# hguo/ftk

Measured on NVIDIA B200. Metric: space_time_simplices_tested_per_sec, higher is better.
Workload: dtype f64+int64

## Files before the change

### ftk_b200/csrc/context.cpp

```cpp
#include <algorithm>
#include <cfloat>
#include <chrono>
#include <cmath>
#include <cstdio>
#include <cstdlib>
#include <cstring>
#include <deque>
#include <string>
#include <thread>
#include <atomic>
#include <vector>

#include <future>
#include <memory>
#include "kernels.h"
#include "online.h"
#include "curves.h"

using namespace ftkb;

namespace {

thread_local std::string g_create_error;

// ... 19 lines not shown
};
template <class T> using RawVec = std::vector<T, NoInitAlloc<T>>;

struct ftkb_ctx {
  ftkb_config cfg{};
  int n = 0;
  size_t nvert = 0;
  uint64_t ncore = 0;
  int n_ord = 0, n_int = 0;
  cudaStream_t stream = nullptr;
  cudaEvent_t ev[8] = {nullptr, nullptr, nullptr, nullptr, nullptr, nullptr, nullptr, nullptr};
  bool derive_timed = false;
  std::string error;

  bool slab = false;
  void *d_f32 = nullptr;
  size_t f32_cap = 0;
  std::deque<Layer> layers;
  std::vector<double *> freeS, freeV, freeJ;
  int current_timestep = 0;
  double resolution = DBL_MAX;
  double factor = 1.0;
  int nbits = 0;
  int next_slot = 0;
  int sm_count = 148;
  int scan_mode = 2;
  bool cellsV = true;
  bool cells2d = true;
  bool keys2d = true;
  bool cells3d = true;
  std::vector<uint4 *> freeCells;
  std::vector<uint4 *> exportedCells;
  size_t ncells = 0;
  bool fused3d = false;

  unsigned long long *d_scalars = nullptr;
  unsigned long long *h_scalars = nullptr;
  static constexpr int SLOT_WL = 8, SLOT_PT = 9, SLOT_UQ = 10, SLOT_POISON = 11, SLOT_WL2 = 12, SLOT_TICKET = 13, SLOT_POISON2 = 14, NSLOTS = 16;

  struct Pending {
    int ring = 0, evset = 0, pops = 0, nbits = 0, wl_sel = 0;
    uint64_t seq = 0, npts_before = 0, pt_cap = 0;
    bool has_next = false;
    int res_slots[2] = {-1, -1};
  };
  bool defer = true;
  std::deque<Pending> pend;
  std::deque<Layer> limbo;
  unsigned long long *h_ring = nullptr;
  static constexpr int RING = 4;
  uint64_t step_seq = 0;
  bool primed = false;
  int wl_sel = 0;
  cudaEvent_t dev[2][3] = {{nullptr, nullptr, nullptr}, {nullptr, nullptr, nullptr}};
  bool push_d2h_outstanding = false;
  uint64_t wl_hint = 1 << 16;
  cudaEvent_t ev_input = nullptr;
  cudaStream_t producer = nullptr;
  cudaStream_t stream2 = nullptr;
  cudaEvent_t ev_join = nullptr;
  bool debug_timing = false;
  double gap_ms = 0; uint64_t gap_n = 0, last_confirmed_seq = 0;
  std::vector<float> gaps, tl_scan_end, tl_test_end;
  cudaEvent_t dbg_prev = nullptr; bool dbg_prev_valid = false;
  double host_wait_us = 0, host_enq_us = 0; uint64_t host_wait_n = 0, host_enq_n = 0;
  bool overlap_test = true;
// ... 590 lines not shown
static void fused3d_decomposition(const ftkb_ctx *c, SweepParams &p, bool cells = false) {
  p.nsx = (p.W + F3_STRIDE - 1) / F3_STRIDE;
  p.nsy = (p.H + F3_TROWS - 1) / F3_TROWS;
  const int64_t tiles = (int64_t)p.nsx * p.nsy;
  if (c->cells3d || cells) {
    const int64_t slots = 2 * (int64_t)c->sm_count;
    const int64_t nsz = std::max<int64_t>(1, std::min<int64_t>((6 * slots + tiles - 1) / tiles, std::max(1, p.D / 16)));
    p.rows = (int)((p.D + nsz - 1) / nsz);
    if (const char *e = std::getenv("FTKB_S3_ROWS")) p.rows = std::max(1, std::min(p.D, std::atoi(e)));
    p.rows = std::min(p.rows, 63);
    p.nsz = (p.D + p.rows - 1) / p.rows;
    return;
  }
  int64_t nsz = std::max<int64_t>(1, (2 * (int64_t)c->sm_count) / tiles);
  nsz = std::min<int64_t>(nsz, std::max(1, p.D / 8));
  p.rows = (int)((p.D + nsz - 1) / nsz);
  p.nsz = (p.D + p.rows - 1) / p.rows;
}

static void vcells_decomposition(const ftkb_ctx *c, SweepParams &p) {
  if (c->n == 3) { fused3d_decomposition(c, p, true); return; }
  const int R = VSCAN2D_CELL_ROWS;
  p.nsx = std::max(1, (p.W + 61) / 62);
  const int64_t want = std::max<int64_t>(1, (6 * (int64_t)c->sm_count * 16) / p.nsx);
  p.rows = std::max(2 * R, (int)((p.H + want - 1) / want));
  p.rows = (p.rows + R - 1) / R * R;
  if (const char *e = std::getenv("FTKB_V2_ROWS")) p.rows = std::max(R, std::atoi(e) / R * R);
  p.nsy = (p.H + p.rows - 1) / p.rows;
  p.nsz = 1;
}

static int ensure_cells(ftkb_ctx *c, Layer &l, const SweepParams &p) {
  if (l.cells) return FTKB_OK;
  if (!c->ncells) c->ncells = c->n == 3 ? scan3d_cells_per_layer(p) : (p.fused ? scan2d_cells_per_layer(p) : vscan2d_cells_per_layer(p));
  if (!c->freeCells.empty()) { l.cells = c->freeCells.back(); c->freeCells.pop_back(); return FTKB_OK; }
  CK(cudaMalloc(&l.cells, sizeof(uint4) * c->ncells));
  return FTKB_OK;
}

static int materialise_gradient(ftkb_ctx *c, Layer &l) {
  if (l.V || !l.S) return FTKB_OK;
  CK(cudaMemsetAsync(c->d_scalars + l.slot, 0xff, sizeof(unsigned long long), c->stream));
  int rc = take_buffer(c, c->freeV, c->nvert * c->n, &l.V);
  if (rc) return rc;
  l.ownV = true;
  l.cells_valid = false;
  launch_gradient(c->n, l.S, l.V, c->cfg.dims[0], c->cfg.dims[1], c->n == 3 ? c->cfg.dims[2] : 1, c->d_scalars + l.slot, c->stream);
  c->stats.kernel_launches++;
  l.res_pending = false;
  CK(cudaMemcpyAsync(c->h_scalars + l.slot, c->d_scalars + l.slot, sizeof(unsigned long long), cudaMemcpyDeviceToHost, c->stream));
  c->stats.d2h_bytes += 8;
  c->push_d2h_outstanding = true;
  return check_launch(c, "gradient");
}

static int abandon_fused3d(ftkb_ctx *c) {
  c->fused3d = false;
  for (Layer &l : c->layers) {
    const int rc = materialise_gradient(c, l);
    if (rc) return rc;
  }
  CK(cudaStreamSynchronize(c->stream));
  return FTKB_OK;
}

static bool rows_aligned16(const ftkb_ctx *c, const double *a, const double *b) {
  return (c->cfg.dims[0] % 2 == 0) && ((uintptr_t)a % 16 == 0) && (!b || (uintptr_t)b % 16 == 0);
}

// ... 1025 lines not shown
  std::memcpy(out->bytes, &h, 64);
  out->offset = (uint64_t)((uintptr_t)dev_ptr - (uintptr_t)base);
  return FTKB_OK;
}

extern "C" int ftkb_ipc_import(const ftkb_ipc_handle *h, int device, void **dev_ptr) {
  if (!h || !dev_ptr) return FTKB_ERR_INVALID;
  if (cudaSetDevice(device) != cudaSuccess) { cudaGetLastError(); return FTKB_ERR_NO_DEVICE; }
  cudaIpcMemHandle_t ih;
  std::memcpy(&ih, h->bytes, 64);
  void *base = nullptr;
  if (cudaIpcOpenMemHandle(&base, ih, cudaIpcMemLazyEnablePeerAccess) != cudaSuccess) { cudaGetLastError(); return FTKB_ERR_CUDA; }
  *dev_ptr = static_cast<char *>(base) + h->offset;
  return FTKB_OK;
}

extern "C" int ftkb_ipc_close(void *dev_ptr, const ftkb_ipc_handle *h) {
  if (!dev_ptr || !h) return FTKB_ERR_INVALID;
  if (cudaIpcCloseMemHandle(static_cast<char *>(dev_ptr) - h->offset) != cudaSuccess) { cudaGetLastError(); return FTKB_ERR_CUDA; }
  return FTKB_OK;
}

extern "C" int ftkb_export_layer_cells(ftkb_ctx *c, int index, void **cells, uint64_t *bytes, double *resolution) {
  if (!c || !cells || !bytes) return FTKB_ERR_INVALID;
  if (index < 0 || (size_t)index >= c->layers.size()) return fail(c, FTKB_ERR_INVALID, "export_layer_cells: no such resident layer");
  { const int rc = drain(c); if (rc) return rc; }
  if ((size_t)index >= c->layers.size()) return fail(c, FTKB_ERR_INVALID, "export_layer_cells: no such resident layer");
  Layer &l = c->layers[index];
  if (!l.cells || !l.cells_valid) return fail(c, FTKB_ERR_INVALID, "export_layer_cells: the layer has no range cells yet (a sweep must have read it)");
  CK(cudaSetDevice(c->cfg.device));
  CK(cudaStreamSynchronize(c->stream));
  if (!l.cells_foreign) { l.cells_foreign = true; c->exportedCells.push_back(l.cells); }
  *cells = l.cells;
  *bytes = (uint64_t)c->ncells * sizeof(uint4);
  if (resolution) *resolution = l.res_pending ? DBL_MAX : slot_value(c, l.slot);
  return FTKB_OK;
}

extern "C" int ftkb_push_snapshot_remote(ftkb_ctx *c, const double *scalar, const double *vector, const void *cells, double resolution) {
  if (!c || !cells || (!scalar && !vector)) return FTKB_ERR_INVALID;
  if (c->cfg.jacobian_source == FTKB_SOURCE_GIVEN) return fail(c, FTKB_ERR_INVALID, "push_snapshot_remote: a GIVEN jacobian cannot be remote");
  if (c->cfg.vector_source == FTKB_SOURCE_GIVEN ? !vector : !scalar) return fail(c, FTKB_ERR_INVALID, "push_snapshot_remote: the field the sweep reads is missing");
  CK(cudaSetDevice(c->cfg.device));
  if ((uintptr_t)scalar % 8 != 0 || (uintptr_t)vector % 8 != 0 || (uintptr_t)cells % 16 != 0)
    return fail(c, FTKB_ERR_INVALID, "push_snapshot_remote: arrays must be 8-byte aligned, cells 16-byte aligned");
  Layer l;
  int rc = new_layer(c, l);
  if (rc) return rc;
  l.S = const_cast<double *>(scalar);
  l.V = const_cast<double *>(vector);
  l.cells = reinterpret_cast<uint4 *>(const_cast<void *>(cells));
  l.cells_valid = true;
  l.cells_foreign = true;
  l.res_pending = false;
  unsigned long long bits;
  const double r = resolution > 0 ? resolution : DBL_MAX;
  std::memcpy(&bits, &r, 8);
  if (!(resolution > 0) || resolution >= DBL_MAX) bits = ~0ull;
  c->h_scalars[l.slot] = bits;
  CK(cudaMemcpyAsync(c->d_scalars + l.slot, c->h_scalars + l.slot, sizeof(unsigned long long), cudaMemcpyHostToDevice, c->stream));
  c->layers.push_back(l);
  return FTKB_OK;
}

extern "C" int ftkb_get_curveset(ftkb_ctx *c, ftkb_curveset **out) {
  if (!c || !out) return FTKB_ERR_INVALID;
  if (!c->traced) return fail(c, FTKB_ERR_INVALID, "get_curveset: call finalize first");
// ... 203 lines not shown
```

### ftk_b200/csrc/kernels.cu

```cuda
#include "kernels.h"

#include <algorithm>
#include <cfloat>
#include <cstdlib>
#include <string>
#include <climits>
#include <cub/device/device_radix_sort.cuh>
#include <cub/device/device_select.cuh>

namespace ftkb {

typedef long long i64;
typedef unsigned long long u64;

__constant__ DeviceMeshTables c_mesh[2];

void upload_mesh_tables(const DeviceMeshTables &t2, const DeviceMeshTables &t3) {
  DeviceMeshTables h[2] = {t2, t3};
  cudaMemcpyToSymbol(c_mesh, h, sizeof(h));
}

constexpr int KEY_ONE = 0x3FF00000;
constexpr int KEY_POISON_EXP = 0x43E00000;

// ... 758 lines not shown
      const int col_lo = max(C0 - 2, 0), col_hi = min(C0 - 2 + TL_SEG, W);
      const uint32_t seg_bytes = (uint32_t)(col_hi - col_lo) * 8u;
      const uint32_t dst0 = smem_u32(ring) + (uint32_t)(col_lo - (C0 - 2)) * 8u;
      for (int rr = 0; rr < nrows; rr++) {
        const int st = rr % TL_NST;
        if (rr >= TL_NST) mbar_wait(empty0 + 8u * st, (uint32_t)((rr / TL_NST - 1) & 1));
        const size_t off = (size_t)W * (size_t)clampi(r0 - 1 + rr, H) + (size_t)col_lo;
        mbar_expect_tx(full0 + 8u * st, seg_bytes * NL);
#pragma unroll
        for (int L = 0; L < NL; L++)
          bulk_g2s(dst0 + (uint32_t)st * STAGE_BYTES + (uint32_t)(L * TL_SEG) * 8u, (L == 0 ? p.L[0].S : p.L[1].S) + off, seg_bytes, full0 + 8u * st);
      }
    }
    return;
  }
  if (wib >= nactive) return;
  const int c0 = C0 + wib * FB_STRIDE;
  const double *tile = ring + wib * FB_STRIDE;
  const bool border = c0 == 0 || c0 + FB_SEG - 2 > W || (p.ub[0] >= c0 - 1 && p.ub[0] <= c0 + 63);
  if (border) fused2d_tile_strip<HAS_NEXT, true>(p, c0, r0, r1, lane, tile, full0, empty0);
  else fused2d_tile_strip<HAS_NEXT, false>(p, c0, r0, r1, lane, tile, full0, empty0);
}

constexpr int C2_R = 9;
constexpr int C2_NST = 9;
constexpr int C2_CW = TL_CW;
static_assert(C2_R % 3 == 0 && C2_R == C2_NST && C2_R == SCAN2D_CELL_ROWS, "row window / ring / cell block must stay aligned");

__device__ __forceinline__ size_t cells2d_index(const SweepParams &p, const int strip, const int kb, const int lane) {
  const size_t nblk = (size_t)(p.H / C2_R + 2);
  return ((size_t)strip * nblk + (size_t)kb) * 32u + (size_t)lane;
}

template <int NL>
__device__ __forceinline__ void cells2d_slow_cubes_t(const SweepParams &p, unsigned failmask, const int c0, const int y0, const int nrows, const uint32_t stage) {
  static_assert(2 * C2_R <= 32, "one lane per cube");
  const int W = p.W, H = p.H;
  const int lane = threadIdx.x & 31;
  const float cwf = (float)(W - 1), chf = (float)(H - 1);
  const float nanf_ = __int_as_float(0x7FC00000);
  const int per = 2 * nrows, total = per * __popc(failmask);
  for (int q0 = 0; q0 < total; q0 += 32) {
    const int qi = q0 + lane;
    const bool live = qi < total;
    const int which = live ? qi / per : 0, within = live ? qi % per : 0;
    const int src = (int)__fns(failmask, 0, which + 1);
    const int r = within >> 1, q = within & 1;
    const int x = c0 + 2 * src + q, y = y0 + r;
    const bool in = live && x >= p.lb[0] && x <= p.ub[0] && y >= p.lb[1] && y <= p.ub[1];
    const int xs[4] = {clampi(x - 1, W), clampi(x, W), clampi(x + 1, W), clampi(x + 2, W)};
    size_t rows_[4];
#pragma unroll
    for (int k = 0; k < 4; k++) rows_[k] = (size_t)W * (size_t)clampi(y - 1 + k, H);
    FRange rx{nanf_, nanf_}, ry{nanf_, nanf_};
#pragma unroll
    for (int L = 0; L < NL; L++) {
      const double *S = p.L[L].S;
      double h[2][4], lo[2], hi[2];
#pragma unroll
      for (int j = 0; j < 2; j++)
#pragma unroll
        for (int k = 0; k < 4; k++) h[j][k] = __ldg(S + rows_[1 + j] + xs[k]);
#pragma unroll
      for (int i = 0; i < 2; i++) { lo[i] = __ldg(S + rows_[0] + xs[1 + i]); hi[i] = __ldg(S + rows_[3] + xs[1 + i]); }
#pragma unroll
      for (int v = 0; v < 4; v++) {
// ... 5 lines not shown
        rx = fmerge(rx, FRange{fx, fx}); ry = fmerge(ry, FRange{fy, fy});
      }
    }
    const bool surv = in && !cube_excluded2_f(rx, ry, p.thrp_f, p.thr2_f, p.lim_f);
    const u64 lin = (u64)(x - p.lb[0]) + (u64)p.nc[0] * (u64)(y - p.lb[1]);
    if (stage) stage_survivors(p, stage, surv, lin);
    else append_survivors(p, surv, lin);
  }
}
__device__ __noinline__ void cells2d_slow_cubes(const SweepParams &p, unsigned failmask, const int c0, const int y0, const int nl, const int nrows, const uint32_t stage = 0) {
  if (nl == 1) cells2d_slow_cubes_t<1>(p, failmask, c0, y0, nrows, stage);
  else cells2d_slow_cubes_t<2>(p, failmask, c0, y0, nrows, stage);
}

__device__ __forceinline__ void cells2d_decide(const SweepParams &p, const FRange ux, const FRange uy, const bool own, const int e, const int y0, const int nl) {
  const bool fail = own && !cube_excluded2_f(ux, uy, p.thrp_f, p.thr2_f, p.lim_f);
  const unsigned fm = __ballot_sync(0xffffffffu, fail);
  if (fm) cells2d_slow_cubes(p, fm, e - 2 * (int)(threadIdx.x & 31), y0, nl, C2_R);
}

template <bool BORDER, int NPREV, bool TEST>
__device__ __forceinline__ void cells2d_strip(const SweepParams &p, const int c0, const int r0, const int r1, const int lane,
                                              const double *tile , const uint32_t full0, const uint32_t empty0,
                                              const int strip) {
  const int W = p.W, H = p.H, B = p.build_layer;
  const int e = c0 + 2 * lane, o = e + 1;
  const bool e_in = !BORDER || e < W, o_in = !BORDER || o < W, o1_in = !BORDER || o + 1 < W;
  const bool own_cols = lane <= 30 && ((e >= p.lb[0] && e <= p.ub[0]) || (o >= p.lb[0] && o <= p.ub[0]));
  const int jl = r1 + 1;
  const float cwf = (float)(W - 1), chf = (float)(H - 1);
  const bool want_res = p.res_slot[B] != nullptr;
  double rmin = DBL_MAX;
  float rminf = 3.4028234e38f;
  const uint4 *sum_prev = NPREV ? p.sum_in[0] + cells2d_index(p, strip, 0, lane) : nullptr;
  uint4 *sum_out = p.sum_out + cells2d_index(p, strip, 0, lane);

  const double *lane_base = tile + 2 * lane;
  auto centre = [&](const int st, double (&dst)[2]) {
    const double2 t = *reinterpret_cast<const double2 *>(lane_base + st * TL_SEG + 2);
    dst[0] = t.x; dst[1] = t.y;
  };
  auto release = [&](const int st) {
    __syncwarp();
    if (elect_one()) mbar_arrive(empty0 + 8u * st);
  };
  auto finish_block = [&](const int kb, FRange bx, FRange by, const uint4 prevc) {
    bx = fmerge(bx, fshfl_down1(bx));
    by = fmerge(by, fshfl_down1(by));
    sum_out[(size_t)kb * 32u] = make_uint4(__float_as_uint(bx.mn), __float_as_uint(bx.mx), __float_as_uint(by.mn), __float_as_uint(by.mx));
    if (TEST) {
      if (NPREV) {
        bx = fmerge(bx, FRange{__uint_as_float(prevc.x), __uint_as_float(prevc.y)});
        by = fmerge(by, FRange{__uint_as_float(prevc.z), __uint_as_float(prevc.w)});
      }
      const int y0 = kb * C2_R;
      const bool own = own_cols && y0 <= p.ub[1] && y0 + C2_R - 1 >= p.lb[1];
      cells2d_decide(p, bx, by, own, e, y0, NPREV + 1);
    }
  };

  double win[3][2];
  mbar_wait(full0, 0);
  centre(0, win[0]);
  mbar_wait(full0 + 8, 0);
  centre(1, win[1]);
  release(0);
  FRange bx{0.f, 0.f}, by{0.f, 0.f};
  uint4 prevc = make_uint4(0x7FC00000u, 0x7FC00000u, 0x7FC00000u, 0x7FC00000u);

  auto step = [&](auto KC, const int j, const int i) {
    constexpr int K = decltype(KC)::value;
    constexpr int ST_J = (1 + K) % C2_NST, ST_P = (2 + K) % C2_NST;
    double (&m1)[2] = win[K % 3];
    double (&c0v)[2] = win[(K + 1) % 3];
    double (&p1)[2] = win[(K + 2) % 3];
    mbar_wait(full0 + 8u * ST_P, (uint32_t)((i + (2 + K >= C2_NST ? 1 : 0)) & 1));
    centre(ST_P, p1);
    const double *rowj = lane_base + ST_J * TL_SEG;
    double left = rowj[1], right = rowj[4];
    double mid_e = c0v[1];
    if (BORDER) {
      if (e == 0) left = c0v[0];
      if (!o_in) mid_e = c0v[0];
      if (!o1_in) right = c0v[1];
    }
    const double dxe = mid_e - left, dxo = right - c0v[0], dye = p1[0] - m1[0], dyo = p1[1] - m1[1];
    const float fxe = __double2float_rn(dxe) * cwf, fxo = __double2float_rn(dxo) * cwf;
    const float fye = __double2float_rn(dye) * chf, fyo = __double2float_rn(dyo) * chf;
    if (want_res && j < H) {
      float a = fminf(fminf(fabsf(fxe), fabsf(fye)), fminf(fabsf(fxo), fabsf(fyo)));
      if (BORDER) a = fminf(e_in ? fminf(fabsf(fxe), fabsf(fye)) : 3.4028234e38f, o_in ? fminf(fabsf(fxo), fabsf(fyo)) : 3.4028234e38f);
      if (a < rminf) res_update4(rmin, rminf, e_in, o_in, dxe, dye, dxo, dyo, (double)(W - 1), (double)(H - 1));
    }
    const FRange rx{fminf(fxe, fxo), fmaxf(fxe, fxo)}, ry{fminf(fye, fyo), fmaxf(fye, fyo)};
    if (K == 0) {
      if (j > r0) finish_block(j / C2_R - 1, fmerge(bx, rx), fmerge(by, ry), prevc);
      bx = rx; by = ry;
      if (NPREV && j < jl) prevc = __ldg(sum_prev + (size_t)(j / C2_R) * 32u);
    } else {
      bx = fmerge(bx, rx); by = fmerge(by, ry);
    }
// ... 44 lines not shown
      const uint32_t seg_bytes = (uint32_t)(col_hi - col_lo) * 8u;
      const uint32_t dst0 = smem_u32(ring) + (uint32_t)(col_lo - (C0 - 2)) * 8u;
      for (int rr = 0; rr < nrows; rr++) {
        const int st = rr % C2_NST;
        if (rr >= C2_NST) mbar_wait(empty0 + 8u * st, (uint32_t)((rr / C2_NST - 1) & 1));
        const size_t off = (size_t)W * (size_t)clampi(r0 - 1 + rr, H) + (size_t)col_lo;
        mbar_expect_tx(full0 + 8u * st, seg_bytes);
        bulk_g2s(dst0 + (uint32_t)st * STAGE_BYTES, S + off, seg_bytes, full0 + 8u * st);
      }
    }
    return;
  }
  if (wib >= nactive) return;
  const int c0 = C0 + wib * FB_STRIDE;
  const double *tile = ring + wib * FB_STRIDE;
  const bool border = c0 == 0 || c0 + FB_SEG - 2 > W;
  if (border) cells2d_strip<true, NPREV, TEST>(p, c0, r0, r1, lane, tile, full0, empty0, bx * C2_CW + wib);
  else cells2d_strip<false, NPREV, TEST>(p, c0, r0, r1, lane, tile, full0, empty0, bx * C2_CW + wib);
}

template <int NL>
__global__ void __launch_bounds__(256) scan2d_cells_kernel(const __grid_constant__ SweepParams p, const int nstrips, const int nblk_used) {
  const int lane = threadIdx.x & 31;
  const long long w = (long long)blockIdx.x * 8 + (threadIdx.x >> 5);
  if (w >= (long long)nstrips * nblk_used) return;
  const int strip = (int)(w / nblk_used), kb = (int)(w % nblk_used);
  const int e = strip * FB_STRIDE + 2 * lane, y0 = kb * C2_R;
  const bool own = lane <= 30 && ((e >= p.lb[0] && e <= p.ub[0]) || (e + 1 >= p.lb[0] && e + 1 <= p.ub[0])) && y0 <= p.ub[1] && y0 + C2_R - 1 >= p.lb[1];
  if (!__any_sync(0xffffffffu, own)) return;
  const float nanf_ = __int_as_float(0x7FC00000);
  FRange ux{nanf_, nanf_}, uy{nanf_, nanf_};
#pragma unroll
  for (int L = 0; L < NL; L++) {
    const uint4 c = __ldg(p.sum_in[L] + cells2d_index(p, strip, kb, lane));
    ux = fmerge(ux, FRange{__uint_as_float(c.x), __uint_as_float(c.y)});
    uy = fmerge(uy, FRange{__uint_as_float(c.z), __uint_as_float(c.w)});
  }
  cells2d_decide(p, ux, uy, own, e, y0, NL);
}

constexpr int K2_R = 3;
constexpr uint32_t K2_ROW_BYTES = TL_SEG * 8;
constexpr uint32_t K2_STAGE_BYTES = K2_R * K2_ROW_BYTES;
static_assert(C2_R % K2_R == 0, "cell block = whole stages");

__device__ __forceinline__ double2 lds128_f64(uint32_t a) {
  double2 v;
  asm volatile("ld.shared.v2.f64 {%0, %1}, [%2];" : "=d"(v.x), "=d"(v.y) : "r"(a));
  return v;
}
__device__ __forceinline__ double lds64_f64(uint32_t a) {
  double v;
  asm volatile("ld.shared.f64 %0, [%1];" : "=d"(v) : "r"(a));
  return v;
}
__device__ __forceinline__ void cp_async16(uint32_t dst, const void *src) {
  asm volatile("cp.async.cg.shared.global [%0], [%1], 16;" ::"r"(dst), "l"(src) : "memory");
}
__device__ __forceinline__ void cp_async_wait_all() { asm volatile("cp.async.wait_all;" ::: "memory"); }
__device__ __forceinline__ void cp_async_commit() { asm volatile("cp.async.commit_group;" ::: "memory"); }
template <int N> __device__ __forceinline__ void cp_async_wait_group() { asm volatile("cp.async.wait_group %0;" ::"n"(N) : "memory"); }
__device__ __forceinline__ uint4 lds128_u32(uint32_t a) {
  uint4 v;
  asm volatile("ld.shared.v4.u32 {%0, %1, %2, %3}, [%4];" : "=r"(v.x), "=r"(v.y), "=r"(v.z), "=r"(v.w) : "r"(a) : "memory");
  return v;
}
__device__ __forceinline__ void sts64_f64(uint32_t a, double v) { asm volatile("st.shared.f64 [%0], %1;" ::"r"(a), "d"(v) : "memory"); }
__device__ __forceinline__ float fmax_nan(float a, float b) {
  float r;
  asm("max.NaN.f32 %0, %1, %2;" : "=f"(r) : "f"(a), "f"(b));
  return r;
}

__device__ __forceinline__ double nzmin(double m, double d) {
  double r;
  asm("{\n\t.reg .pred p, q;\n\t.reg .f64 ad, am;\n\tabs.f64 ad, %2;\n\tabs.f64 am, %1;\n\t"
      "setp.neu.f64 q, %2, 0d0000000000000000;\n\tsetp.lt.and.f64 p, ad, am, q;\n\tselp.f64 %0, %2, %1, p;\n\t}"
      : "=d"(r) : "d"(m), "d"(d));
  return r;
}

__device__ __forceinline__ FRange k2_vrange(float kmn, float kmx, double c) {
  const int a = __float_as_int(kmn), b = __float_as_int(kmx);
  const double lo = __hiloint2double(a < 0 ? a + 1 : a, 0);
  const double hi = __hiloint2double(b < 0 ? b : b + 1, 0);
  return FRange{__double2float_rd(lo * c), __double2float_ru(hi * c)};
}

__device__ __forceinline__ void prefetch_l2(const void *q) { asm volatile("prefetch.global.L2 [%0];" ::"l"(q)); }

struct K2Acc { double mdx, mdy; float big; };

template <bool BORDER, int NPREV, bool TEST, int K2_NST>
__device__ __forceinline__ K2Acc keys2d_strip(const SweepParams &p, const int c0, const int r0, const int r1, const int lane,
                                           const uint32_t tile_u32 ,
                                           const uint32_t full0, const uint32_t empty0, const int strip,
                                           const uint32_t sbase ,
                                           const uint32_t res_u32 ,
                                           const uint32_t wl_stage ,
                                           const uint32_t cell_stage ,
                                           const K2Acc acc) {
  float big = acc.big;
  const int W = p.W, H = p.H, B = p.build_layer;
  const int e = c0 + 2 * lane, o = e + 1;
  const bool e_in = !BORDER || e < W, o_in = !BORDER || o < W, o1_in = !BORDER || o + 1 < W;
  const bool own_cols = lane <= 30 && ((e >= p.lb[0] && e <= p.ub[0]) || (o >= p.lb[0] && o <= p.ub[0]));
  const int jl = r1 + 1;
  const int nrows = jl - r0 + 1;
  const int ngroups = (nrows + K2_R - 1) / K2_R, nstages = (nrows + 2 + K2_R - 1) / K2_R;
  const double cw = (double)(W - 1), ch = (double)(H - 1);
  const bool want_res = p.res_slot[B] != nullptr;
  const float thrx = p.res_thr[0], thry = p.res_thr[1];
  const uint4 *sum_prev = NPREV ? p.sum_in[0] + cells2d_index(p, strip, 0, lane) : nullptr;
  uint4 *sum_out = p.sum_out + cells2d_index(p, strip, 0, lane);
  const uint32_t lane_u32 = tile_u32 + (uint32_t)lane * 16u;
  const int kb0 = r0 / C2_R;
  unsigned long long failbits = 0;
  const int kb_end = ((r1 + 1) + C2_R - 1) / C2_R;

  auto finish_block = [&](const int kb, float xmn, float xmx, float ymn, float ymx) {
    xmn = fminf(xmn, __shfl_down_sync(0xffffffffu, xmn, 1)); xmx = fmaxf(xmx, __shfl_down_sync(0xffffffffu, xmx, 1));
    ymn = fminf(ymn, __shfl_down_sync(0xffffffffu, ymn, 1)); ymx = fmaxf(ymx, __shfl_down_sync(0xffffffffu, ymx, 1));
    FRange bx = k2_vrange(xmn, xmx, cw), by = k2_vrange(ymn, ymx, ch);
    sum_out[(size_t)kb * 32u] = make_uint4(__float_as_uint(bx.mn), __float_as_uint(bx.mx), __float_as_uint(by.mn), __float_as_uint(by.mx));
    if (TEST) {
      if (NPREV && kb < kb_end) {
        cp_async_wait_all();
        const uint4 prevc = lds128_u32(cell_stage + ((uint32_t)kb & 1u) * 512u);
        bx = fmerge(bx, FRange{__uint_as_float(prevc.x), __uint_as_float(prevc.y)});
        by = fmerge(by, FRange{__uint_as_float(prevc.z), __uint_as_float(prevc.w)});
      }
      const int y0 = kb * C2_R;
      const bool own = own_cols && y0 <= p.ub[1] && y0 + C2_R - 1 >= p.lb[1];
      if (own && !cube_excluded2_f(bx, by, p.thrp_f, p.thr2_f, p.lim_f)) failbits |= 1ull << (kb - kb0);
    }
  };

  double C[2][K2_R][2];
  float KX[2][K2_R][2];
  auto load_stage = [&](auto PC, const int s) {
    constexpr int P = decltype(PC)::value;
    const uint32_t gs = sbase + (uint32_t)s, slot = gs % K2_NST;
    mbar_wait(full0 + 8u * slot, (gs / K2_NST) & 1u);
    const uint32_t base = lane_u32 + slot * K2_STAGE_BYTES;
    double nl[K2_R], nr[K2_R];
#pragma unroll
    for (int i = 0; i < K2_R; i++) {
      const double2 c = lds128_f64(base + (uint32_t)i * K2_ROW_BYTES + 16u);
      C[P][i][0] = c.x; C[P][i][1] = c.y;
      nl[i] = lds64_f64(base + (uint32_t)i * K2_ROW_BYTES + 8u);
      nr[i] = lds64_f64(base + (uint32_t)i * K2_ROW_BYTES + 32u);
    }
    float ax = __int_as_float(0x7F800000);
#pragma unroll
    for (int i = 0; i < K2_R; i++) {
      const float ke = fabsf(hikey(C[P][i][0])), ko = fabsf(hikey(C[P][i][1]));
      big = fmax_nan(big, BORDER ? (e_in ? ke : 0.f) : ke);
      big = fmax_nan(big, BORDER ? (o_in ? ko : 0.f) : ko);
      double left = nl[i], right = nr[i], mid_e = C[P][i][1];
      if (BORDER) {
        if (e == 0) left = C[P][i][0];
        if (!o_in) mid_e = C[P][i][0];
        if (!o1_in) right = C[P][i][1];
      }
      const double dxe = mid_e - left, dxo = right - C[P][i][0];
      KX[P][i][0] = hikey(dxe); KX[P][i][1] = hikey(dxo);
      ax = fminf(ax, fminf(fabsf(KX[P][i][0]), fabsf(KX[P][i][1])));
    }
    if (want_res && __any_sync(0xffffffffu, ax <= thrx)) {
      double mdx = lds64_f64(res_u32);
#pragma unroll
      for (int i = 0; i < K2_R; i++) {
        const int j = r0 + K2_R * s + i - 1;
        if (j >= r0 && j <= jl && j < H) {
          double left = lds64_f64(base + (uint32_t)i * K2_ROW_BYTES + 8u), right = lds64_f64(base + (uint32_t)i * K2_ROW_BYTES + 32u), mid_e = C[P][i][1];
          if (BORDER) {
            if (e == 0) left = C[P][i][0];
            if (!o_in) mid_e = C[P][i][0];
            if (!o1_in) right = C[P][i][1];
          }
          if (e_in) mdx = nzmin(mdx, mid_e - left);
          if (o_in) mdx = nzmin(mdx, right - C[P][i][0]);
        }
      }
      sts64_f64(res_u32, mdx);
    }
    __syncwarp();
    if (elect_one()) mbar_arrive(empty0 + 8u * slot);
  };

  float bxmn = 0.f, bxmx = 0.f, bymn = 0.f, bymx = 0.f;
  const uint4 nanc = make_uint4(0x7FC00000u, 0x7FC00000u, 0x7FC00000u, 0x7FC00000u);
  int kb = r0 / C2_R;
  if (NPREV && kb < kb_end) prefetch_l2(sum_prev + (size_t)kb * 32u);
  if (NPREV && kb + 1 < kb_end) prefetch_l2(sum_prev + (size_t)(kb + 1) * 32u);

  int gphase = 0;
  static_assert(C2_R == 3 * K2_R, "a cell block is three groups");
  auto group = [&](auto PC, const int g) {
    constexpr int P = decltype(PC)::value;
    if (g + 1 < nstages) load_stage(IC<1 - P>{}, g + 1);
    const bool opens_group = gphase == 0;
    gphase = gphase == 2 ? 0 : gphase + 1;
    const int j0 = r0 + K2_R * g;
    const bool full = j0 + K2_R - 1 <= min(jl, H - 1);
    float ay = __int_as_float(0x7F800000);
#pragma unroll
    for (int i = 0; i < K2_R; i++) {
      const int j = j0 + i;
      if (!full && j > jl) break;
      const double *m1 = C[P][i];
      const float *kx = i + 1 < K2_R ? KX[P][i + 1] : KX[1 - P][i + 1 - K2_R];
      const double *p1 = i + 2 < K2_R ? C[P][i + 2] : C[1 - P][i + 2 - K2_R];
      const double dye = p1[0] - m1[0], dyo = p1[1] - m1[1];
      const float kxe = kx[0], kxo = kx[1], kye = hikey(dye), kyo = hikey(dyo);
      ay = fminf(ay, fminf(fabsf(kye), fabsf(kyo)));
      if (i == 0 && opens_group) {
        const float rxmn = fminf(kxe, kxo), rxmx = fmaxf(kxe, kxo), rymn = fminf(kye, kyo), rymx = fmaxf(kye, kyo);
        if (j > r0) finish_block(kb - 1, fminf(bxmn, rxmn), fmaxf(bxmx, rxmx), fminf(bymn, rymn), fmaxf(bymx, rymx));
        bxmn = rxmn; bxmx = rxmx; bymn = rymn; bymx = rymx;
        if (NPREV && kb < kb_end) cp_async16(cell_stage + ((uint32_t)kb & 1u) * 512u, sum_prev + (size_t)kb * 32u);
        kb++;
        if (NPREV && kb + 1 < kb_end) prefetch_l2(sum_prev + (size_t)(kb + 1) * 32u);
      } else {
        bxmn = fminf(fminf(bxmn, kxe), kxo); bxmx = fmaxf(fmaxf(bxmx, kxe), kxo);
        bymn = fminf(fminf(bymn, kye), kyo); bymx = fmaxf(fmaxf(bymx, kye), kyo);
      }
    }
    if (want_res && __any_sync(0xffffffffu, ay <= thry)) {
      double mdy = lds64_f64(res_u32 + 8u);
#pragma unroll
      for (int i = 0; i < K2_R; i++) {
        const int j = j0 + i;
        if (!full && (j > jl || j >= H)) break;
        const double *m1 = C[P][i];
        const double *p1 = i + 2 < K2_R ? C[P][i + 2] : C[1 - P][i + 2 - K2_R];
        if (e_in) mdy = nzmin(mdy, p1[0] - m1[0]);
        if (o_in) mdy = nzmin(mdy, p1[1] - m1[1]);
      }
      sts64_f64(res_u32 + 8u, mdy);
    }
  };

  load_stage(IC<0>{}, 0);
#pragma unroll 1
  for (int g = 0; g < ngroups; g += 2) {
    group(IC<0>{}, g);
    if (g + 1 < ngroups) group(IC<1>{}, g + 1);
  }
  if (jl % C2_R != 0) finish_block(jl / C2_R, bxmn, bxmx, bymn, bymx);
  if (TEST) {
    for (int b = 0; b < 64; b++) {
      if (!__any_sync(0xffffffffu, (failbits >> b) != 0)) break;
      const unsigned fm = __ballot_sync(0xffffffffu, (failbits >> b) & 1ull);
// ... 75 lines not shown
    const char *e = std::getenv("FTKB_K2_CTAS"), *n = std::getenv("FTKB_K2_NST");
    const int ctas = e ? std::atoi(e) : 3, nst = n ? std::atoi(n) : 4;
    if (ctas == 2) return 28;
    if (ctas == 4) return 44;
    return nst == 5 ? 35 : (nst == 6 ? 36 : 34);
  }();
  return v;
}
template <int CTAS, int NST>
static void k2_launch(const SweepParams &p, unsigned grid, cudaStream_t s) {
  const size_t sm = k2_smem_bytes(NST);
  switch (p.sum_mode) {
    case SUM_BUILD: scan2d_keys_build_kernel<0, false, CTAS, NST><<<grid, (C2_CW + 1) * 32, sm, s>>>(p); break;
    case SUM_BUILD_TEST1: scan2d_keys_build_kernel<0, true, CTAS, NST><<<grid, (C2_CW + 1) * 32, sm, s>>>(p); break;
    default: scan2d_keys_build_kernel<1, true, CTAS, NST><<<grid, (C2_CW + 1) * 32, sm, s>>>(p); break;
  }
}
template <int CTAS, int NST>
static void k2_attrs() {
  const int sm = (int)k2_smem_bytes(NST);
  cudaFuncSetAttribute(scan2d_keys_build_kernel<0, false, CTAS, NST>, cudaFuncAttributeMaxDynamicSharedMemorySize, sm);
  cudaFuncSetAttribute(scan2d_keys_build_kernel<0, true, CTAS, NST>, cudaFuncAttributeMaxDynamicSharedMemorySize, sm);
  cudaFuncSetAttribute(scan2d_keys_build_kernel<1, true, CTAS, NST>, cudaFuncAttributeMaxDynamicSharedMemorySize, sm);
}

static size_t c2_smem_bytes() { return (size_t)C2_NST * TL_SEG * 8 + (size_t)2 * C2_NST * 8; }

size_t vscan2d_cells_per_layer(const SweepParams &p);
void launch_scan2d_direct(const SweepParams &p, cudaStream_t s);
size_t scan2d_cells_per_layer(const SweepParams &p) {
  if (p.bulk == 3) return vscan2d_cells_per_layer(p);
  return (size_t)p.nsx * C2_CW * (size_t)(p.H / C2_R + 2) * 32u;
}

void launch_scan2d_cells(const SweepParams &p, cudaStream_t s) {
  if (p.bulk == 3) { launch_scan2d_direct(p, s); return; }
  const unsigned grid = (unsigned)((i64)p.nsx * p.nsy);
  const int nstrips = (p.W + FB_STRIDE - 1) / FB_STRIDE, nblk = (p.H + C2_R - 1) / C2_R;
  const unsigned tgrid = (unsigned)(((i64)nstrips * nblk + 7) / 8);
  if (p.keys2d && p.sum_mode <= SUM_BUILD_TEST2) {
    switch (k2_variant()) {
      case 28: k2_launch<2, 8>(p, grid, s); break;
      case 44: k2_launch<4, 4>(p, grid, s); break;
      case 35: k2_launch<3, 5>(p, grid, s); break;
      case 36: k2_launch<3, 6>(p, grid, s); break;
      default: k2_launch<3, 4>(p, grid, s); break;
    }
    return;
  }
  switch (p.sum_mode) {
    case SUM_BUILD: scan2d_build_kernel<0, false><<<grid, (C2_CW + 1) * 32, c2_smem_bytes(), s>>>(p); break;
    case SUM_BUILD_TEST1: scan2d_build_kernel<0, true><<<grid, (C2_CW + 1) * 32, c2_smem_bytes(), s>>>(p); break;
    case SUM_BUILD_TEST2: scan2d_build_kernel<1, true><<<grid, (C2_CW + 1) * 32, c2_smem_bytes(), s>>>(p); break;
    case SUM_TEST1: scan2d_cells_kernel<1><<<tgrid, 256, 0, s>>>(p, nstrips, nblk); break;
    default: scan2d_cells_kernel<2><<<tgrid, 256, 0, s>>>(p, nstrips, nblk); break;
  }
}

constexpr int F3_LAYER_BYTES = ((F3_ROWS * F3_COLS * 8 + 127) / 128) * 128;
constexpr int F3_LAYER_DOUBLES = F3_LAYER_BYTES / 8;
constexpr uint32_t F3_BOX_BYTES = F3_ROWS * F3_COLS * 8;

__device__ __forceinline__ void tma_load_3d(uint32_t dst, const CUtensorMap *tm, int c0, int c1, int c2, uint32_t bar) {
  asm volatile("cp.async.bulk.tensor.3d.shared::cluster.global.tile.mbarrier::complete_tx::bytes [%0], [%1, {%2, %3, %4}], [%5];"
               ::"r"(dst), "l"(tm), "r"(c0), "r"(c1), "r"(c2), "r"(bar) : "memory");
}
// ... 2297 lines not shown
```

### ftk_b200/csrc/kernels.h

```cpp
#pragma once
#include <cuda.h>
#include <cuda_runtime.h>
#include <cstdint>

#include "../../include/ftkb200.h"
#include "mesh_tables.h"

namespace ftkb {

struct LayerPtrs {
  const double *S;
  const double *V;
  const double *J;
};

struct SweepParams {
  int32_t nd;
  int32_t W, H, D;
  int32_t lb[3], ub[3];
  int32_t nc[3];
  int32_t vmax[3];
  int32_t voff[3], rank_lb[3], rank_nc[3];
  int32_t t;
  int32_t has_next;
// ... 45 lines not shown
  if (!(R < 0x1p1000) || !(scale > 0.0)) return __builtin_inff();
  const double T = R / scale;
  unsigned long long bits;
  __builtin_memcpy(&bits, &T, 8);
  const int hi = (int)(bits >> 32) + 2;
  float f;
  __builtin_memcpy(&f, &hi, 4);
  return f;
}

void upload_mesh_tables(const DeviceMeshTables &t2, const DeviceMeshTables &t3);
void init_kernel_attributes();

constexpr int F3_CW = 8;
constexpr int F3_RW = 4;
constexpr int F3_NST = 5;
constexpr int F3_STRIDE = 62;
constexpr int F3_COLS = 68;
constexpr int F3_TROWS = F3_CW * F3_RW;
constexpr int F3_ROWS = F3_TROWS + 3;
bool encode_scalar_tmap3d(const double *S, int W, int H, int D, CUtensorMap *out);

void launch_scan(const SweepParams &p, cudaStream_t s);
enum { SUM_BUILD = 0,
       SUM_BUILD_TEST1 = 1,
       SUM_BUILD_TEST2 = 2,
       SUM_TEST1 = 3,
       SUM_TEST2 = 4 };
void launch_scan3d_cells(const SweepParams &p, cudaStream_t s);
size_t scan3d_cells_per_layer(const SweepParams &p);
constexpr int SCAN2D_CELL_ROWS = 9;
void launch_scan2d_cells(const SweepParams &p, cudaStream_t s);
size_t scan2d_cells_per_layer(const SweepParams &p);
constexpr int VSCAN2D_CELL_ROWS = 8;
void launch_vscan_cells(const SweepParams &p, cudaStream_t s);
size_t vscan2d_cells_per_layer(const SweepParams &p);
void launch_test(const SweepParams &p, cudaStream_t s);

void launch_gradient(int nd, const double *S, double *V, int W, int H, int D, unsigned long long *res_bits, cudaStream_t s);
void launch_resolution(const double *p, uint64_t n, unsigned long long *res_bits, cudaStream_t s);
void launch_fill_u64(unsigned long long *p, unsigned long long v, cudaStream_t s);
void launch_widen_f32(const float *in, double *out, uint64_t n, cudaStream_t s);

void launch_synthetic(int kind, int nd, int W, int H, int D, const double *params, double t, double *out, cudaStream_t s, int zoff = 0, int Dg = 0);

struct TraceParams {
  int32_t nd;
  int32_t lb[3], ub[3];
  int64_t ny, nz;
  uint64_t n;
  const unsigned long long *keys;
  const ftkb_point *pts;
  uint32_t *nb;
  int32_t *deg;
  uint32_t *parent_all;
  uint32_t *parent_ord;
};
constexpr int KEY_TYPE_BITS = 6;
constexpr int KEY_TIME_BITS = 22;

void launch_point_keys(const ftkb_point *pts, uint64_t n, const TraceParams &tp, unsigned long long *keys, uint32_t *idx, cudaStream_t s);
void launch_gather_points(const ftkb_point *src, const uint32_t *idx, uint64_t n, ftkb_point *dst, cudaStream_t s);
void launch_neighbors(const TraceParams &tp, cudaStream_t s);
void launch_union_find(const TraceParams &tp, cudaStream_t s);
void launch_batch_neighbors(const TraceParams &tp, const unsigned long long *n_ptr, uint64_t n_max, const ftkb_point *src, const uint32_t *idx,
                            ftkb_point *dst, uint32_t *nb9, uint8_t *cnt, cudaStream_t s);
// ... 8 lines not shown
```

Baseline: 5527 billion.

## Compress 2D range cells to 64-bit quantized encoding with shared exponent

Replaces the 16-byte float range summary per 2D cell block with an 8-byte encoding: a shared 8-bit exponent and four 14-bit outwardly rounded fixed-point bounds. Writers encode and readers decode, the async staging copy drops to 8 bytes, and allocation and export sizes follow a per-context cell byte size. The aim is to halve the memory traffic for cell summaries written and reread across layers. Decoded ranges are conservative, so they only widen, which may send more cubes down the slow path, and the encode and decode add ALU work.

```diff
diff --git a/ftk_b200/csrc/context.cpp b/ftk_b200/csrc/context.cpp
--- a/ftk_b200/csrc/context.cpp
+++ b/ftk_b200/csrc/context.cpp
@@ -75,6 +75,7 @@
   std::vector<uint4 *> freeCells;
   std::vector<uint4 *> exportedCells;
   size_t ncells = 0;
+  size_t cell_bytes = 0;
   bool fused3d = false;
 
   unsigned long long *d_scalars = nullptr;
@@ -731,9 +732,12 @@
 
 static int ensure_cells(ftkb_ctx *c, Layer &l, const SweepParams &p) {
   if (l.cells) return FTKB_OK;
-  if (!c->ncells) c->ncells = c->n == 3 ? scan3d_cells_per_layer(p) : (p.fused ? scan2d_cells_per_layer(p) : vscan2d_cells_per_layer(p));
+  if (!c->ncells) {
+    c->ncells = c->n == 3 ? scan3d_cells_per_layer(p) : (p.fused ? scan2d_cells_per_layer(p) : vscan2d_cells_per_layer(p));
+    c->cell_bytes = c->n == 2 && p.fused ? scan2d_cell_bytes(p) : sizeof(uint4);
+  }
   if (!c->freeCells.empty()) { l.cells = c->freeCells.back(); c->freeCells.pop_back(); return FTKB_OK; }
-  CK(cudaMalloc(&l.cells, sizeof(uint4) * c->ncells));
+  CK(cudaMalloc(&l.cells, c->cell_bytes * c->ncells));
   return FTKB_OK;
 }
 
@@ -1825,7 +1829,7 @@
   CK(cudaStreamSynchronize(c->stream));
   if (!l.cells_foreign) { l.cells_foreign = true; c->exportedCells.push_back(l.cells); }
   *cells = l.cells;
-  *bytes = (uint64_t)c->ncells * sizeof(uint4);
+  *bytes = (uint64_t)c->ncells * c->cell_bytes;
   if (resolution) *resolution = l.res_pending ? DBL_MAX : slot_value(c, l.slot);
   return FTKB_OK;
 }
diff --git a/ftk_b200/csrc/kernels.cu b/ftk_b200/csrc/kernels.cu
--- a/ftk_b200/csrc/kernels.cu
+++ b/ftk_b200/csrc/kernels.cu
@@ -814,6 +814,28 @@
   return ((size_t)strip * nblk + (size_t)kb) * 32u + (size_t)lane;
 }
 
+__device__ __forceinline__ uint2 cell2d_encode(const FRange x, const FRange y) {
+  const float m = fmaxf(fmaxf(fabsf(x.mn), fabsf(x.mx)), fmaxf(fabsf(y.mn), fabsf(y.mx)));
+  if (isnan(x.mn) || isnan(x.mx) || isnan(y.mn) || isnan(y.mx) || !(m <= 3.4028234e38f)) return make_uint2(0xFFu, 0u);
+  const uint32_t E = max((__float_as_uint(m) >> 23) & 0xFFu, 12u);
+  const float up = __uint_as_float((265u - E) << 23);
+  const uint32_t a = (uint32_t)(int)floorf(__fmul_rd(x.mn, up)) & 0x3FFFu, b = (uint32_t)(int)ceilf(__fmul_ru(x.mx, up)) & 0x3FFFu;
+  const uint32_t c = (uint32_t)(int)floorf(__fmul_rd(y.mn, up)) & 0x3FFFu, d = (uint32_t)(int)ceilf(__fmul_ru(y.mx, up)) & 0x3FFFu;
+  return make_uint2(E | a << 8 | b << 22, b >> 10 | c << 4 | d << 18);
+}
+__device__ __forceinline__ void cell2d_decode(const uint2 w, FRange &x, FRange &y) {
+  const uint32_t E = w.x & 0xFFu;
+  if (E == 0xFFu) {
+    const float inf = __int_as_float(0x7F800000);
+    x = y = FRange{-inf, inf};
+    return;
+  }
+  const float u = __uint_as_float((E - 11u) << 23);
+  auto q = [&](const uint32_t bits14) { return (float)((int)(bits14 << 18) >> 18) * u; };
+  x = FRange{q((w.x >> 8) & 0x3FFFu), q((w.x >> 22 | w.y << 10) & 0x3FFFu)};
+  y = FRange{q((w.y >> 4) & 0x3FFFu), q((w.y >> 18) & 0x3FFFu)};
+}
+
 template <int NL>
 __device__ __forceinline__ void cells2d_slow_cubes_t(const SweepParams &p, unsigned failmask, const int c0, const int y0, const int nrows, const uint32_t stage) {
   static_assert(2 * C2_R <= 32, "one lane per cube");
@@ -885,8 +907,8 @@
   const bool want_res = p.res_slot[B] != nullptr;
   double rmin = DBL_MAX;
   float rminf = 3.4028234e38f;
-  const uint4 *sum_prev = NPREV ? p.sum_in[0] + cells2d_index(p, strip, 0, lane) : nullptr;
-  uint4 *sum_out = p.sum_out + cells2d_index(p, strip, 0, lane);
+  const uint2 *sum_prev = NPREV ? reinterpret_cast<const uint2 *>(p.sum_in[0]) + cells2d_index(p, strip, 0, lane) : nullptr;
+  uint2 *sum_out = reinterpret_cast<uint2 *>(p.sum_out) + cells2d_index(p, strip, 0, lane);
 
   const double *lane_base = tile + 2 * lane;
   auto centre = [&](const int st, double (&dst)[2]) {
@@ -897,14 +919,16 @@
     __syncwarp();
     if (elect_one()) mbar_arrive(empty0 + 8u * st);
   };
-  auto finish_block = [&](const int kb, FRange bx, FRange by, const uint4 prevc) {
+  auto finish_block = [&](const int kb, FRange bx, FRange by, const uint2 prevc) {
     bx = fmerge(bx, fshfl_down1(bx));
     by = fmerge(by, fshfl_down1(by));
-    sum_out[(size_t)kb * 32u] = make_uint4(__float_as_uint(bx.mn), __float_as_uint(bx.mx), __float_as_uint(by.mn), __float_as_uint(by.mx));
+    sum_out[(size_t)kb * 32u] = cell2d_encode(bx, by);
     if (TEST) {
       if (NPREV) {
-        bx = fmerge(bx, FRange{__uint_as_float(prevc.x), __uint_as_float(prevc.y)});
-        by = fmerge(by, FRange{__uint_as_float(prevc.z), __uint_as_float(prevc.w)});
+        FRange px, py;
+        cell2d_decode(prevc, px, py);
+        bx = fmerge(bx, px);
+        by = fmerge(by, py);
       }
       const int y0 = kb * C2_R;
       const bool own = own_cols && y0 <= p.ub[1] && y0 + C2_R - 1 >= p.lb[1];
@@ -919,7 +943,7 @@
   centre(1, win[1]);
   release(0);
   FRange bx{0.f, 0.f}, by{0.f, 0.f};
-  uint4 prevc = make_uint4(0x7FC00000u, 0x7FC00000u, 0x7FC00000u, 0x7FC00000u);
+  uint2 prevc = make_uint2(0xFFu, 0u);
 
   auto step = [&](auto KC, const int j, const int i) {
     constexpr int K = decltype(KC)::value;
@@ -1030,9 +1054,10 @@
   FRange ux{nanf_, nanf_}, uy{nanf_, nanf_};
 #pragma unroll
   for (int L = 0; L < NL; L++) {
-    const uint4 c = __ldg(p.sum_in[L] + cells2d_index(p, strip, kb, lane));
-    ux = fmerge(ux, FRange{__uint_as_float(c.x), __uint_as_float(c.y)});
-    uy = fmerge(uy, FRange{__uint_as_float(c.z), __uint_as_float(c.w)});
+    FRange cx, cy;
+    cell2d_decode(__ldg(reinterpret_cast<const uint2 *>(p.sum_in[L]) + cells2d_index(p, strip, kb, lane)), cx, cy);
+    ux = fmerge(ux, cx);
+    uy = fmerge(uy, cy);
   }
   cells2d_decide(p, ux, uy, own, e, y0, NL);
 }
@@ -1054,6 +1079,9 @@
 }
 __device__ __forceinline__ void cp_async16(uint32_t dst, const void *src) {
   asm volatile("cp.async.cg.shared.global [%0], [%1], 16;" ::"r"(dst), "l"(src) : "memory");
+}
+__device__ __forceinline__ void cp_async8(uint32_t dst, const void *src) {
+  asm volatile("cp.async.ca.shared.global [%0], [%1], 8;" ::"r"(dst), "l"(src) : "memory");
 }
 __device__ __forceinline__ void cp_async_wait_all() { asm volatile("cp.async.wait_all;" ::: "memory"); }
 __device__ __forceinline__ void cp_async_commit() { asm volatile("cp.async.commit_group;" ::: "memory"); }
@@ -1061,6 +1089,11 @@
 __device__ __forceinline__ uint4 lds128_u32(uint32_t a) {
   uint4 v;
   asm volatile("ld.shared.v4.u32 {%0, %1, %2, %3}, [%4];" : "=r"(v.x), "=r"(v.y), "=r"(v.z), "=r"(v.w) : "r"(a) : "memory");
+  return v;
+}
+__device__ __forceinline__ uint2 lds64_u32(uint32_t a) {
+  uint2 v;
+  asm volatile("ld.shared.v2.u32 {%0, %1}, [%2];" : "=r"(v.x), "=r"(v.y) : "r"(a) : "memory");
   return v;
 }
 __device__ __forceinline__ void sts64_f64(uint32_t a, double v) { asm volatile("st.shared.f64 [%0], %1;" ::"r"(a), "d"(v) : "memory"); }
@@ -1109,8 +1142,8 @@
   const double cw = (double)(W - 1), ch = (double)(H - 1);
   const bool want_res = p.res_slot[B] != nullptr;
   const float thrx = p.res_thr[0], thry = p.res_thr[1];
-  const uint4 *sum_prev = NPREV ? p.sum_in[0] + cells2d_index(p, strip, 0, lane) : nullptr;
-  uint4 *sum_out = p.sum_out + cells2d_index(p, strip, 0, lane);
+  const uint2 *sum_prev = NPREV ? reinterpret_cast<const uint2 *>(p.sum_in[0]) + cells2d_index(p, strip, 0, lane) : nullptr;
+  uint2 *sum_out = reinterpret_cast<uint2 *>(p.sum_out) + cells2d_index(p, strip, 0, lane);
   const uint32_t lane_u32 = tile_u32 + (uint32_t)lane * 16u;
   const int kb0 = r0 / C2_R;
   unsigned long long failbits = 0;
@@ -1120,13 +1153,14 @@
     xmn = fminf(xmn, __shfl_down_sync(0xffffffffu, xmn, 1)); xmx = fmaxf(xmx, __shfl_down_sync(0xffffffffu, xmx, 1));
     ymn = fminf(ymn, __shfl_down_sync(0xffffffffu, ymn, 1)); ymx = fmaxf(ymx, __shfl_down_sync(0xffffffffu, ymx, 1));
     FRange bx = k2_vrange(xmn, xmx, cw), by = k2_vrange(ymn, ymx, ch);
-    sum_out[(size_t)kb * 32u] = make_uint4(__float_as_uint(bx.mn), __float_as_uint(bx.mx), __float_as_uint(by.mn), __float_as_uint(by.mx));
+    sum_out[(size_t)kb * 32u] = cell2d_encode(bx, by);
     if (TEST) {
       if (NPREV && kb < kb_end) {
         cp_async_wait_all();
-        const uint4 prevc = lds128_u32(cell_stage + ((uint32_t)kb & 1u) * 512u);
-        bx = fmerge(bx, FRange{__uint_as_float(prevc.x), __uint_as_float(prevc.y)});
-        by = fmerge(by, FRange{__uint_as_float(prevc.z), __uint_as_float(prevc.w)});
+        FRange px, py;
+        cell2d_decode(lds64_u32(cell_stage + ((uint32_t)kb & 1u) * 512u), px, py);
+        bx = fmerge(bx, px);
+        by = fmerge(by, py);
       }
       const int y0 = kb * C2_R;
       const bool own = own_cols && y0 <= p.ub[1] && y0 + C2_R - 1 >= p.lb[1];
@@ -1188,7 +1222,6 @@
   };
 
   float bxmn = 0.f, bxmx = 0.f, bymn = 0.f, bymx = 0.f;
-  const uint4 nanc = make_uint4(0x7FC00000u, 0x7FC00000u, 0x7FC00000u, 0x7FC00000u);
   int kb = r0 / C2_R;
   if (NPREV && kb < kb_end) prefetch_l2(sum_prev + (size_t)kb * 32u);
   if (NPREV && kb + 1 < kb_end) prefetch_l2(sum_prev + (size_t)(kb + 1) * 32u);
@@ -1217,7 +1250,7 @@
         const float rxmn = fminf(kxe, kxo), rxmx = fmaxf(kxe, kxo), rymn = fminf(kye, kyo), rymx = fmaxf(kye, kyo);
         if (j > r0) finish_block(kb - 1, fminf(bxmn, rxmn), fmaxf(bxmx, rxmx), fminf(bymn, rymn), fmaxf(bymx, rymx));
         bxmn = rxmn; bxmx = rxmx; bymn = rymn; bymx = rymx;
-        if (NPREV && kb < kb_end) cp_async16(cell_stage + ((uint32_t)kb & 1u) * 512u, sum_prev + (size_t)kb * 32u);
+        if (NPREV && kb < kb_end) cp_async8(cell_stage + ((uint32_t)kb & 1u) * 512u, sum_prev + (size_t)kb * 32u);
         kb++;
         if (NPREV && kb + 1 < kb_end) prefetch_l2(sum_prev + (size_t)(kb + 1) * 32u);
       } else {
@@ -1359,6 +1392,7 @@
   if (p.bulk == 3) return vscan2d_cells_per_layer(p);
   return (size_t)p.nsx * C2_CW * (size_t)(p.H / C2_R + 2) * 32u;
 }
+size_t scan2d_cell_bytes(const SweepParams &p) { return p.bulk == 3 ? sizeof(uint4) : sizeof(uint2); }
 
 void launch_scan2d_cells(const SweepParams &p, cudaStream_t s) {
   if (p.bulk == 3) { launch_scan2d_direct(p, s); return; }
diff --git a/ftk_b200/csrc/kernels.h b/ftk_b200/csrc/kernels.h
--- a/ftk_b200/csrc/kernels.h
+++ b/ftk_b200/csrc/kernels.h
@@ -101,6 +101,7 @@
 constexpr int SCAN2D_CELL_ROWS = 9;
 void launch_scan2d_cells(const SweepParams &p, cudaStream_t s);
 size_t scan2d_cells_per_layer(const SweepParams &p);
+size_t scan2d_cell_bytes(const SweepParams &p);
 constexpr int VSCAN2D_CELL_ROWS = 8;
 void launch_vscan_cells(const SweepParams &p, cudaStream_t s);
 size_t vscan2d_cells_per_layer(const SweepParams &p);
```

Measured after the change: 5539 billion (median of 6 runs). Within noise of the previous version (+0.2%).
